# re-ovo/wgpu-path-tracing

Measured on AMD Instinct MI355X. Metric: Msamples/s (rays x bounces / s), higher is better.
Workload: dtype f32

## Files before the change

### include/ptmi.h

```cpp
#ifndef PTMI_H
#define PTMI_H

#include <stddef.h>
#include <stdint.h>
#include "ptmi_layout.h"

#ifdef __cplusplus
extern "C" {
#endif

#define PTMI_ABI_VERSION 4

enum {
    PTMI_OK = 0,
    PTMI_E_INVALID = -1,
    PTMI_E_NODEVICE = -2,
    PTMI_E_HIP = -3,
    PTMI_E_STATE = -4,
    PTMI_E_UNSUPPORTED = -5
};

enum { PTMI_ATLAS_RGBA16F = 1, PTMI_ATLAS_RGBA32F = 2 };
enum { PTMI_TRAVERSAL_AUTO = 0, PTMI_TRAVERSAL_GLOBAL = 1, PTMI_TRAVERSAL_LDS = 2, PTMI_TRAVERSAL_GLOBAL_EXACT = 3 };

// ... 370 lines not shown
int ptmi_multi_alpha_status(ptmi_multi *m, struct ptmi_alpha_status *out);

typedef struct ptmi_alpha_blend_params {
    uint32_t max_layers;
    uint32_t seed;
    uint32_t reserved[2];
} ptmi_alpha_blend_params;
struct ptmi_alpha_blend_status {
    uint32_t present, n_materials, n_blend, max_layers, seed, reserved;
    uint64_t path_tests, path_passes, shadow_tests, shadow_passes;
};
int ptmi_set_alpha_blend(ptmi_ctx *ctx, const float *factor, uint32_t n_materials, const ptmi_alpha_blend_params *params );
int ptmi_alpha_blend_status(ptmi_ctx *ctx, struct ptmi_alpha_blend_status *out);
int ptmi_multi_set_alpha_blend(ptmi_multi *m, const float *factor, uint32_t n_materials, const ptmi_alpha_blend_params *params);
int ptmi_multi_alpha_blend_status(ptmi_multi *m, struct ptmi_alpha_blend_status *out);

int ptmi_get_stats(ptmi_ctx *ctx, ptmi_stats *out);
int ptmi_reset_stats(ptmi_ctx *ctx);

int ptmi_debug_raygen(ptmi_ctx *ctx, const ptmi_camera *camera, uint32_t n, const uint32_t *xs,
                      const uint32_t *ys, const uint32_t *frames, float *o3, float *d3, uint32_t *rng);
int ptmi_debug_center_rays(ptmi_ctx *ctx, const ptmi_camera *camera, float *o3, float *d3, size_t n_floats_each);
int ptmi_debug_intersect(ptmi_ctx *ctx, uint32_t n, const float *o3, const float *d3,
                         float *t, uint32_t *tri, float *u, float *v);
int ptmi_debug_occluded(ptmi_ctx *ctx, uint32_t n, const float *o3, const float *d3,
                        const float *dist, uint8_t *occluded);
int ptmi_debug_alpha_intersect(ptmi_ctx *ctx, uint32_t n, const float *o3, const float *d3, float *t, uint32_t *tri, uint32_t *layers);
int ptmi_debug_alpha_occluded(ptmi_ctx *ctx, uint32_t n, const float *o3, const float *d3, const float *dist, uint8_t *occluded,
                              uint32_t *layers);
int ptmi_debug_image_stats(const ptmi_triangle *triangles, uint32_t n_triangles,
// ... 33 lines not shown
```

### wgpu-path-tracing_amd/csrc/dispatch.hip

```cpp
#include "ptmi_ctx.h"

#include <algorithm>
#include <cmath>
#include <cstring>
#include <utility>
#include <vector>

namespace {

constexpr size_t kMaxPendingEvents = 4096;
constexpr size_t kMaxDispatchesInFlight = 256;

const struct { double ptmi_stats::*ms; uint64_t ptmi_stats::*launches; } kEventStat[kEventKinds] = {
    {&ptmi_stats::gpu_ms, nullptr},
    {&ptmi_stats::extend_ms, &ptmi_stats::extend_launches},
    {&ptmi_stats::shade_ms, &ptmi_stats::shade_launches},
    {&ptmi_stats::shadow_ms, &ptmi_stats::shadow_launches},
    {&ptmi_stats::raygen_ms, nullptr},
    {&ptmi_stats::compact_ms, nullptr},
    {&ptmi_stats::accumulate_ms, nullptr},
};

hipEvent_t get_event(ptmi_ctx *c) {
    if (!c->event_pool.empty()) { hipEvent_t e = c->event_pool.back(); c->event_pool.pop_back(); return e; }
// ... 50 lines not shown
}

struct Timed {
    ptmi_ctx *c; hipEvent_t a = nullptr, b = nullptr; EventKind kind; bool on;
    hipStream_t st;
    Timed(ptmi_ctx *c_, EventKind kind_, bool on_, hipStream_t st_ = nullptr) : c(c_), kind(kind_), on(on_), st(st_ ? st_ : c_->stream) {
        if (on) { a = get_event(c); b = get_event(c); (void)hipEventRecord(a, st); }
    }
    ~Timed() {
        if (!on) return;
        (void)hipEventRecord(b, st);
        c->pending.push_back({a, b, kind});
        if (c->pending.size() > kMaxPendingEvents) drain_completed_events(c);
    }
};

#ifndef PT_REPACK
#define PT_REPACK 1
#endif

int dispatch(ptmi_ctx *c, const ptmi_camera *cam, uint32_t n_frames, const ptmi_adaptive_params *ap, uint32_t rounds,
             const DevFlagMap *map = nullptr, bool count_call = true, const ListedRays *listed = nullptr) {
    int rc = check_ready(c, true);
    if (rc) return rc;
    uint32_t proj = PTMI_PROJ_PERSPECTIVE;
    if (!listed) {
        if (!cam) return fail(c, PTMI_E_INVALID, "camera is NULL");
        if (cam->width != c->W || cam->height != c->H)
            return fail(c, PTMI_E_INVALID, "camera says %ux%u but the output buffer is %ux%u", cam->width, cam->height, c->W, c->H);
        if ((rc = pt_check_camera(c, cam, &proj, c->err))) return rc;
// ... 27 lines not shown
    if (npix * F > 0xFFFFFF00ull) return fail(c, PTMI_E_UNSUPPORTED, "batch of %llu paths exceeds 2^32", (unsigned long long)(npix * F));
    TraverseConfig cfg, cfg_shadow;
    if ((rc = traverse_pick(c, true, cfg)) || (rc = traverse_pick(c, false, cfg_shadow))) return rc;
    for (;;) {
        rc = ensure_capacity(c, ln, (size_t)(npix * F), depth);
        if (rc == PTMI_OK) break;
        if (!auto_F || !c->alloc_oom || F <= 1) return rc;
        F = (F + 1) / 2;
    }
    if ((rc = traverse_arm(c, true, kSpillMain, cfg, true)) || (rc = traverse_arm(c, false, side ? kSpillSide : kSpillAfterExtend, cfg_shadow, true)))
        return rc;
    c->st.traversal_used = pt_variant(cfg.variant).where == PT_FROM_MEMORY ? PTMI_TRAVERSAL_GLOBAL : PTMI_TRAVERSAL_LDS;
    c->st.frames_per_batch_used = F;
    c->st.radiance_stride_bytes = (walks_memory_quantised(cfg) || walks_memory_quantised(cfg_shadow)) ? 16u : 12u;
    c->st.shade_tables = PT_SHADE_LDS_BUDGET | ((uint32_t)pt_shade_stage(c->sc.n_mats, c->sc.n_lights) << 28);
    const int blocks = c->n_cu * 8;
#ifndef PT_SHADE_WGS_PER_CU
#define PT_SHADE_WGS_PER_CU 16
#endif
    const int shade_blocks = c->n_cu * PT_SHADE_WGS_PER_CU;
    const uint32_t maxb = c->opt.max_bounces;
    const bool t1 = c->opt.timing >= 1, t2 = c->opt.timing >= 2, t3 = c->opt.timing >= 3;
    {
        Timed td(c, kDispatch, t1);
        const hipStream_t ms = c->stream;
        const hipStream_t ss = side ? ln.side : ms;
        const int tiles = (int)(ln.cap / pt_compact_tile_slots() + 1);
        ln.paths.l_stride = c->st.radiance_stride_bytes / 4u;
        DevPaths bp = ln.paths;
        if (!env_w) bp.W = nullptr;
        const uint32_t rb = PT_REPACK ? pt_repack_bounce() : 0xFFFFFFFEu;
        DevPaths tp = ln.tail;
        tp.L = bp.L; tp.l_stride = bp.l_stride;
        if (!env_w) tp.W = nullptr;
        float4 *const aov_rec = c->aov_mask || depth ? ln.aov : nullptr;
        float4 *const mom = plane_as<float4>(c, kMoments);
        unsigned long long *const ct = c->d_counters;
        uint32_t *const qlen = &c->d_control[kCwQueue], *const slen = &c->d_control[kCwShadow];
        if (ap && !map && first_frame == 0u) { pt_launch_adaptive_restart(ms, blocks, band, mom); c->ad_rounds = 0; }
        const DevRays rays = listed ? listed->rays : DevRays{CameraSource{cam, proj}};
        auto batch = [&](uint32_t frame0, uint32_t fb) -> int {
            const DevPixels px = ap     ? DevPixels{ListedPixels{band, c->ad.list, &c->d_control[kCwAdActive], mom, &ct[kCtAdTraced]}}
                                 : listed ? DevPixels{BakedPixels{band, listed->list, listed->count, frame0}}
                                          : DevPixels{DensePixels{band, frame0}};
            { Timed t(c, kRaygen, t3, ms); pt_launch_raygen(ms, blocks, rays, px, fb, bp, &qlen[0]); }
            int cur = 0;
            for (uint32_t b = 0; b < maxb; b++) {
                const bool tail = b > rb;
                const uint32_t *q = b == 0 || b == rb + 1 ? nullptr : ln.queue[cur];
                const DevPaths sp = tail ? tp : bp;
                const int par = side ? (int)(b & 1u) : 0;
                const ShadeParams shp{b, maxb, c->opt.do_mis, ln.counts, side ? 1u : 0u, tail ? ln.pid : nullptr};
                { Timed t(c, kExtend, t2, ms); launch_extend(c, ms, cfg, sp, q, &qlen[b], ln.hits);
                  if (alpha) alpha_resolve_paths(c, ms, cfg, sp, q, &qlen[b], ln.hits, nullptr); }
                const bool last = b + 1 == maxb;
                if (side && b >= 2) HIP_TRY(c, hipStreamWaitEvent(ms, ln.ev_shadow[par], 0));
                { Timed t(c, kShade, t3, ms);
                  (c->opt.perf_mode ? pt_launch_shade_fast : pt_launch_shade)(
// ... 37 lines not shown
            }
            c->ad_rounds += rounds;
        } else {
            for (uint32_t f0 = 0; f0 < n_frames; f0 += F)
                if ((rc = batch(first_frame + f0, std::min(F, n_frames - f0)))) return rc;
        }
    }
    HIP_TRY(c, hipGetLastError());
    {
        hipEvent_t done = get_event(c);
        HIP_TRY(c, hipEventRecord(done, c->stream));
        c->in_flight.push_back(done);
        if (c->in_flight.size() > kMaxDispatchesInFlight) HIP_TRY(c, throttle(c, kMaxDispatchesInFlight));
    }
    if (!ap) { c->st.paths += npix * n_frames; c->st.frames += n_frames; }
    if (count_call) c->st.dispatches += 1;
    return PTMI_OK;
}

}

int pt_adaptive_check(ptmi_ctx *c, const ptmi_camera *cam, const ptmi_adaptive_params *params, ptmi_adaptive_params *out) {
    if (!c) return PTMI_E_INVALID;
    if (!params) return fail(c, PTMI_E_INVALID, "params is NULL");
    ptmi_adaptive_params ap = *params;
    if (!(ap.threshold > 0.0f)) return fail(c, PTMI_E_INVALID, "threshold %g is not > 0", (double)ap.threshold);
    if (!(ap.floor >= 0.0f) || std::isinf(ap.floor)) return fail(c, PTMI_E_INVALID, "floor %g is negative or not finite", (double)ap.floor);
    if (ap.reserved[0] || ap.reserved[1]) return fail(c, PTMI_E_INVALID, "a reserved word of ptmi_adaptive_params is not zero");
    if (ap.neighbourhood > 1u) return fail(c, PTMI_E_INVALID, "neighbourhood %u is not 0 or 1", ap.neighbourhood);
    if (ap.floor == 0.0f) ap.floor = 1.0f;
// ... 47 lines not shown
}

int ptmi_dispatch_bake(ptmi_ctx *c, const ptmi_bake_params *params, uint32_t n_frames) {
    ptmi_bake_params bp;
    const int rc = bake_check(c, params, &bp);
    if (rc) return rc;
    const ListedRays listed{BakeSurface{c->d_bake_texels, bp.bias}, c->d_bake_covered, c->bake_covered, bp.first_frame};
    return dispatch(c, nullptr, n_frames, nullptr, 0, nullptr, true, &listed);
}

int ptmi_dispatch_probes(ptmi_ctx *c, const ptmi_probe_params *params, uint32_t n_frames) {
    ListedRays listed;
    const int rc = probes_check(c, params, &listed);
    if (rc) return rc;
    return dispatch(c, nullptr, n_frames, nullptr, 0, nullptr, true, &listed);
}

int ptmi_adaptive_status(ptmi_ctx *c, struct ptmi_adaptive_status *out) {
    if (!c || !out) return PTMI_E_INVALID;
    if (!c->moments_on) return fail(c, PTMI_E_STATE, "the moments plane is off (ptmi_set_moments)");
    if (!c->plane[kMoments]) return fail(c, PTMI_E_STATE, "no output buffer (ptmi_resize)");
    HIP_TRY(c, hipSetDevice(c->device));
    std::memset(out, 0, sizeof *out);
    const DevBand band = pt_band_of(c->opt, c->W, c->H);
    const unsigned long long preset[3] = {0ull, ~0ull, 0ull};
    unsigned long long sum_min_max[3] = {0ull, 0ull, 0ull};
    uint32_t active = 0u;
    HIP_TRY(c, quiesce(c));
    if (band.y0 < band.y1 && band.rows) {
        HIP_TRY(c, hipMemcpyAsync(&c->d_counters[kCtAdSum], preset, sizeof preset, hipMemcpyHostToDevice, c->stream));
// ... 118 lines not shown
```

### wgpu-path-tracing_amd/csrc/pipeline.hip

```cpp
#include "pt_ballot_list.h"
#include "pt_device.h"
#include "pt_math.h"

#include <cstdlib>
#include <type_traits>

namespace {

constexpr int BLOCK = 256;

template <int PROJ>
PT_DEV v3 camera_dir(const ptmi_camera &cam, float px, float py, v3 &org0) {
    float uvx = (px / (float)cam.width) * 2.0f - 1.0f;
    float uvy = (py / (float)cam.height) * 2.0f - 1.0f;
    v3 fw = mk3(cam.forward[0], cam.forward[1], cam.forward[2]);
    v3 rt = mk3(cam.right[0], cam.right[1], cam.right[2]);
    v3 up = mk3(cam.up[0], cam.up[1], cam.up[2]);
    org0 = mk3(cam.position[0], cam.position[1], cam.position[2]);
    if constexpr (PROJ == (int)PTMI_PROJ_ORTHOGRAPHIC) {
        const float ymag = __uint_as_float(cam._p3[1]);
        v3 a = scale3(scale3(scale3(rt, uvx), ymag), cam.aspect);
        v3 b = scale3(scale3(up, uvy), ymag);
        org0 = add3(add3(org0, a), b);
        return normalize3(fw);
// ... 89 lines not shown
    const float4 *__restrict__ probes; uint32_t shift, cols, count;
    PT_DEV void ray(uint32_t x, uint32_t y, uint32_t frame, size_t, v3 &o, v3 &d, uint32_t &rng) const {
        const uint32_t i = (y >> shift) * cols + (x >> shift);
        o = d = mk3(0.0f, 0.0f, 0.0f); rng = 0u;
        if ((x >> shift) >= cols || i >= count) return;
        const float4 p = probes[i];
        if (__float_as_uint(p.w) != 0u) probe_ray(p, 1u << shift, x, y, frame, o, d, rng);
    }
};

template <class Rays, class Pixels>
PT_DEV void raygen(const Rays &rays, const Pixels &px, uint32_t n_frames, DevPaths P, uint32_t *__restrict__ count_out) {
    const DevBand &band = px.band;
    const uint32_t n = px.entries();
    const uint32_t total = n * n_frames;
    if (blockIdx.x == 0 && threadIdx.x == 0) { px.count_paths(total); *count_out = total; }
    for (uint32_t p = blockIdx.x * BLOCK + threadIdx.x; p < total; p += gridDim.x * BLOCK) {
        const uint32_t k = p / n, pix = px.pixel(p - k * n);
        const uint32_t y = band.row_of(pix / band.width), x = pix % band.width;
        const size_t fp = (size_t)y * band.width + x;
        v3 o, d; uint32_t rng;
        rays.ray(x, y, px.first_frame(fp) + k, fp, o, d, rng);
        init_path(P, p, o, d, rng);
    }
}
template <class Rays, class Pixels>
__global__ __launch_bounds__(BLOCK) void k_first_rays(Rays rays, Pixels px, uint32_t n_frames, DevPaths P, uint32_t *__restrict__ count_out) {
    raygen(rays, px, n_frames, P, count_out);
}
template <class Rays>
__global__ __launch_bounds__(BLOCK) void k_first_rays_list(Rays rays, uint32_t width, uint32_t n, const uint32_t *xs, const uint32_t *ys,
// ... 95 lines not shown
        const float t = 1.0f / (float)(frame + 1u);
        for (int i = 0; i < N; i++) acc[i] = mix1(acc[i], x[i], t);
    } else {
        for (int i = 0; i < N; i++) acc[i] = x[i];
    }
}
PT_DEV rgb_sc ld_clamped(const float *__restrict__ L, uint32_t l_stride, size_t p) {
    rgb_sc l;
    if (l_stride == 4u) { const float4 v = reinterpret_cast<const float4 *>(L)[p]; l = rgb_sc{v.x, v.y, v.z}; }
    else l = reinterpret_cast<const rgb_sc *>(L)[p];
    return rgb_sc{min1(l.x, 2.5f), min1(l.y, 2.5f), min1(l.z, 2.5f)};
}

template <class Pixels>
PT_DEV void fold_radiance(const Pixels &px, uint32_t n_frames, const float *__restrict__ L, uint32_t l_stride, float4 *__restrict__ out) {
    const uint32_t n = px.entries();
    for (uint32_t j = blockIdx.x * BLOCK + threadIdx.x; j < n; j += gridDim.x * BLOCK) {
        const size_t oi = px.band.frame_pixel(px.pixel(j));
        const uint32_t frame0 = px.first_frame(oi);
        const float4 o = out[oi];
        float acc[3] = {o.x, o.y, o.z};
        for (uint32_t k = 0; k < n_frames; k++) {
            const rgb_sc c = ld_clamped(L, l_stride, (size_t)k * n + j);
            fold(acc, {c.x, c.y, c.z}, frame0 + k);
        }
        out[oi] = n_frames ? make_float4(acc[0], acc[1], acc[2], 0.0f) : o;
    }
}

template <class Pixels>
PT_DEV void fold_aov(const Pixels &px, uint32_t n_frames, const float4 *__restrict__ rec, const ptmi_triangle *__restrict__ tris,
                     uint32_t n_tris, float4 *__restrict__ albedo, float4 *__restrict__ normal, uint2 *__restrict__ ids) {
    const uint32_t n = px.entries();
    for (uint32_t j = blockIdx.x * BLOCK + threadIdx.x; j < n; j += gridDim.x * BLOCK) {
        const size_t oi = px.band.frame_pixel(px.pixel(j));
        const uint32_t frame0 = px.first_frame(oi);
        const float4 a = albedo ? albedo[oi] : make_float4(0.0f, 0.0f, 0.0f, 0.0f);
        const float4 nm = normal ? normal[oi] : make_float4(0.0f, 0.0f, 0.0f, 0.0f);
// ... 356 lines not shown
        hipLaunchKernelGGL(k_scatter_packed, dim3(tiles), dim3(TILE_WORDS), 0, s, count, shadow_mask, shadow_sums, shadow_queue,
                           shadow_count, st);
}
void pt_launch_repack(hipStream_t s, int blocks, const uint32_t *count, const uint32_t *queue, DevPaths from, DevPaths to,
                      uint32_t *pid) {
    hipLaunchKernelGGL(k_repack, dim3(blocks), dim3(BLOCK), 0, s, count, queue, from, to, pid);
}
void pt_launch_accumulate(hipStream_t s, int blocks, const DevPixels &px, uint32_t n_frames, const float *L, uint32_t l_stride, float4 *out) {
    std::visit([&](auto src) {
        hipLaunchKernelGGL(k_fold_radiance<decltype(src)>, dim3(blocks), dim3(BLOCK), 0, s, src, n_frames, L, l_stride, out);
    }, px);
}
void pt_launch_accumulate_aov(hipStream_t s, int blocks, const DevPixels &px, uint32_t n_frames, const float4 *rec,
                              const ptmi_triangle *tris, uint32_t n_tris, float4 *albedo, float4 *normal, uint2 *ids) {
    std::visit([&](auto src) {
        if constexpr (std::is_same_v<decltype(src), BakedPixels>) abort();
        else hipLaunchKernelGGL(k_fold_aov<decltype(src)>, dim3(blocks), dim3(BLOCK), 0, s, src, n_frames, rec, tris, n_tris, albedo, normal, ids);
    }, px);
}
void pt_launch_accumulate_probe_depth(hipStream_t s, int blocks, const DevPixels &px, uint32_t n_frames, const float4 *rec, float max_distance,
                                      float4 *plane) {
    std::visit([&](auto src) {
        if constexpr (std::is_same_v<decltype(src), BakedPixels>)
            hipLaunchKernelGGL(k_fold_probe_depth<BakedPixels>, dim3(blocks), dim3(BLOCK), 0, s, src, n_frames, rec, max_distance, plane);
        else abort();
    }, px);
}
void pt_launch_accumulate_moments(hipStream_t s, int blocks, const DevPixels &px, uint32_t n_frames, const float *L, uint32_t l_stride,
                                  float4 *mom) {
    std::visit([&](auto src) {
        hipLaunchKernelGGL(k_fold_moments<decltype(src)>, dim3(blocks), dim3(BLOCK), 0, s, src, n_frames, L, l_stride, mom);
    }, px);
}
void pt_launch_adaptive_restart(hipStream_t s, int blocks, DevBand band, float4 *mom) {
    hipLaunchKernelGGL(k_ad_restart, dim3(blocks), dim3(BLOCK), 0, s, band, mom);
}
void pt_launch_adaptive_list(hipStream_t s, int blocks, DevBand band, const ptmi_adaptive_params &ap, const float4 *mom,
                             const DevFlagMap *fm, DevAdaptive ad) {
    const int tiles = (int)pt_adaptive_tiles(band.rows * band.width);
    uint32_t *const n_pixels = &ad.control[kCwAdPixels];
    if (fm) hipLaunchKernelGGL(k_ad_select_map, dim3(blocks), dim3(BLOCK), 0, s, band, ap, mom, *fm, ad.ballot, ad.control);
    else hipLaunchKernelGGL(k_ad_select, dim3(blocks), dim3(BLOCK), 0, s, band, ap, mom, ad.ballot, ad.control);
    hipLaunchKernelGGL(k_ad_tile_sums, dim3(tiles), dim3(TILE_WORDS), 0, s, n_pixels, ad.ballot, ad.tile_sums);
    hipLaunchKernelGGL(k_ad_scatter, dim3(tiles), dim3(TILE_WORDS), 0, s, n_pixels, ad.ballot, ad.tile_sums, ad.list, &ad.control[kCwAdActive]);
}
void pt_launch_adaptive_flags(hipStream_t s, int blocks, DevBand band, const ptmi_adaptive_params &ap, const float4 *mom, uint8_t *flags) {
// ... 22 lines not shown
```

### wgpu-path-tracing_amd/csrc/pt_device.h

```cpp
#pragma once
#include <hip/hip_runtime.h>
#include <stdint.h>
#include <initializer_list>
#include <variant>
#include "ptmi_layout.h"
#include "ptmi.h"

#define PT_HD __host__ __device__ inline

#define PT_REF_LEAF      0x80000000u
#define PT_REF_NONE      0xFFFFFFFFu
#define PT_LEAF_MAX_TRIS 32u
#define PT_LEAF_OFF_BITS 26u
#define PT_LEAF_OFF_MASK ((1u << PT_LEAF_OFF_BITS) - 1u)

struct DevEnv {
    const float4 *tab;
    const uint2 *alias;
    uint32_t w, h;
    uint32_t sampled;
    float intensity, rotation;
};

struct DevMedium {
// ... 203 lines not shown
    int wants_spill;
    int quantized;
};
inline uint32_t pt_variant_code(const TraverseConfig &cfg) { return (uint32_t)cfg.variant * 10u + (uint32_t)cfg.wgs_per_cu; }
#ifndef PT_QCACHE_NODES
#define PT_QCACHE_NODES 256
#endif
#define PT_SPILL_ENTRIES 64
size_t pt_spill_bytes(int blocks);

struct DensePixels {
    DevBand band; uint32_t frame0;
    __device__ uint32_t entries() const { return band.rows * band.width; }
    __device__ uint32_t pixel(uint32_t j) const { return j; }
    __device__ uint32_t first_frame(size_t) const { return frame0; }
    __device__ void count_paths(uint32_t) const {}
};
struct ListedPixels {
    DevBand band; const uint32_t *list, *n_active; const float4 *mom;
    unsigned long long *traced;
    __device__ uint32_t entries() const { return *n_active; }
    __device__ uint32_t pixel(uint32_t j) const { return list[j]; }
    __device__ uint32_t first_frame(size_t oi) const { return (uint32_t)mom[oi].z; }
    __device__ void count_paths(uint32_t paths) const { atomicAdd(traced, (unsigned long long)paths); }
};
struct BakedPixels {
    DevBand band; const uint32_t *covered; uint32_t n, frame0;
    __device__ uint32_t entries() const { return n; }
    __device__ uint32_t pixel(uint32_t j) const { return covered[j]; }
    __device__ uint32_t first_frame(size_t) const { return frame0; }
    __device__ void count_paths(uint32_t) const {}
};
using DevPixels = std::variant<DensePixels, ListedPixels, BakedPixels>;
struct CameraSource { const ptmi_camera *cam; uint32_t proj; };
struct BakeSurface { const float4 *texels; float bias; };
struct ProbeSet { const float4 *probes; uint32_t shift, cols, count; };
using DevRays = std::variant<CameraSource, BakeSurface, ProbeSet>;
void pt_launch_raygen(hipStream_t s, int blocks, const DevRays &rays, const DevPixels &px, uint32_t n_frames, DevPaths p, uint32_t *count_out);
void pt_launch_raygen_list(hipStream_t s, const DevRays &rays, uint32_t width, uint32_t n, const uint32_t *xs, const uint32_t *ys,
                           const uint32_t *frames, DevPaths p);
float4 *pt_launch_bake_dilate(hipStream_t s, uint32_t W, uint32_t H, uint32_t passes, const float4 *texels, const float4 *out,
                              float4 *a, float4 *b);
struct DevProbeAtlas { const float4 *out; const float4 *probes; uint32_t W, shift, cols, count; };
void pt_launch_probe_sh(hipStream_t s, DevProbeAtlas a, const float *basis9, float *sh);
size_t pt_probe_irradiance_lds(uint32_t shift);
void pt_launch_probe_irradiance(hipStream_t s, DevProbeAtlas a, const float4 *dir_dw, const float4 *normals, uint32_t m, float4 *irr);
void pt_launch_probe_visibility(hipStream_t s, DevProbeAtlas depth, const float4 *dir_dw, const float4 *normals, uint32_t m, uint32_t sharpness_log2,
                                uint32_t border, float4 *vis);
// ... 107 lines not shown
```

### wgpu-path-tracing_amd/csrc/ptmi_api.hip

```cpp
#include "ptmi_ctx.h"

#include <algorithm>
#include <cmath>
#include <cstdarg>
#include <cstdio>
#include <cstring>

namespace {

void vfail(std::string &err, const char *fmt, va_list ap) {
    char buf[512];
    vsnprintf(buf, sizeof buf, fmt, ap);
    err = buf;
}

constexpr size_t kLaneBytes[kLaneBufs] = {
    16, 16, 8, 16,
    8,
    16 + 16 + sizeof(rgb_sc), 4, 16 + 16 + sizeof(rgb_sc), 4,
    16, 16, 8, 4,
    4, 4,
    1,
    32,
    4, 4,
// ... 248 lines not shown
#else
        ok = ok && hipStreamCreateWithPriority(&ln.side, hipStreamNonBlocking, hi) == hipSuccess;
#endif
        for (hipEvent_t *e : {&ln.ev_ready, &ln.ev_shadow[0], &ln.ev_shadow[1]})
            ok = ok && hipEventCreateWithFlags(e, hipEventDisableTiming) == hipSuccess;
        if (!ok) { ptmi_destroy(c); return fail(nullptr, PTMI_E_HIP, "stream / event creation failed"); }
    }
    if (hipMalloc(&c->d_counters, kCounterWords * sizeof(unsigned long long)) != hipSuccess ||
        hipMalloc(&c->d_control, kControlWords * sizeof(uint32_t)) != hipSuccess ||
        hipMalloc(&c->d_scene, sizeof(DevScene)) != hipSuccess || hipMemset(c->d_scene, 0, sizeof(DevScene)) != hipSuccess ||
        hipMemset(c->d_counters, 0, kCounterWords * sizeof(unsigned long long)) != hipSuccess ||
        hipMemset(c->d_control, 0, kControlWords * sizeof(uint32_t)) != hipSuccess) {
        ptmi_destroy(c); return fail(nullptr, PTMI_E_HIP, "device allocation failed");
    }
    c->ad.control = c->d_control; c->ad.counters = c->d_counters;
    *out = c;
    return PTMI_OK;
}

int ptmi_destroy(ptmi_ctx *c) {
    if (!c) return PTMI_E_INVALID;
    (void)hipSetDevice(c->device);
    (void)sync_all(c);
    drain_events(c);
    for (hipEvent_t e : c->in_flight) (void)hipEventDestroy(e);
    for (hipEvent_t e : c->event_pool) (void)hipEventDestroy(e);
    {
        Lane &ln = c->lane;
        free_batch(ln);
        dfree(ln.d_spill); dfree(ln.d_spill_side);
// ... 342 lines not shown
    for (int i = 0; i < kMaxBounces; i++) c->st.segments_by_bounce[i] = h[kCtByBounce + i];
    c->st.verify_failed = h[kCtVerifyFailed];
    c->st.bvh_depth = stats_depth(c);
    *out = c->st;
    out->paths += h[kCtAdTraced];
    return PTMI_OK;
}

int ptmi_reset_stats(ptmi_ctx *c) {
    if (!c) return PTMI_E_INVALID;
    HIP_TRY(c, hipSetDevice(c->device));
    HIP_TRY(c, quiesce(c));
    HIP_TRY(c, hipMemset(c->d_counters, 0, kCtDispatchEnd * sizeof(unsigned long long)));
    const ptmi_stats old = c->st;
    std::memset(&c->st, 0, sizeof c->st);
    c->st.bvh_depth = stats_depth(c);
    c->st.upload_ms = old.upload_ms; c->st.upload_tree_ms = old.upload_tree_ms; c->st.upload_copy_ms = old.upload_copy_ms;
    c->st.leaves_used = old.leaves_used; c->st.leaf_tris_used = old.leaf_tris_used; c->st.tree_builder_used = old.tree_builder_used;
    return PTMI_OK;
}

}
```

### wgpu-path-tracing_amd/csrc/ptmi_ctx.h

```cpp
#pragma once
#include "ptmi.h"
#include "pt_device.h"

#include <chrono>
#include <cmath>
#include <cstddef>
#include <cstdint>
#include <deque>
#include <string>
#include <vector>

struct ptmi_ctx;
struct PtPrepared;
PtPrepared *pt_prepare_scene(ptmi_ctx *c, const ptmi_triangle *tris, uint32_t nt, const ptmi_material *mats, uint32_t nm,
                             const ptmi_bvh_node *nodes, uint32_t nn, const ptmi_light *lights, uint32_t nl, int *rc_out);
int pt_install_scene(ptmi_ctx *c, PtPrepared *p);
void pt_free_prepared(PtPrepared *p);
int pt_atlas_bytes(uint32_t width, uint32_t height, int format, size_t *bytes, char *why, size_t why_len);
int pt_check_medium(const ptmi_medium *m, std::string &err);
int pt_check_medium_depth(const ptmi_medium *m, std::string &err);
int pt_check_medium_density(const float *rho, uint32_t nx, uint32_t ny, uint32_t nz, const ptmi_medium_grid *params,
                            struct ptmi_medium_grid_status *st, std::string &err);
const ptmi_medium *pt_ctx_medium(const ptmi_ctx *c);
bool pt_ctx_has_medium_grid(const ptmi_ctx *c);
// ... 174 lines not shown
    uint32_t *d_bake_covered = nullptr;
    uint32_t bake_covered = 0;
    float4 *d_probes = nullptr;
    uint32_t *d_probe_list = nullptr;
    float4 *d_probe_dir_dw = nullptr;
    float *d_probe_basis = nullptr;
    float4 *d_probe_normals = nullptr;
    struct ptmi_probe_status probe{};
    bool probe_depth_on = false;
    ptmi_probe_depth_params probe_depth{};
    unsigned long long *d_counters = nullptr;
    uint32_t *d_control = nullptr;
    DevAdaptive ad{};
    uint32_t ad_rounds = 0;

    ptmi_stats st{};
    std::vector<EventPair> pending;
    std::vector<hipEvent_t> event_pool;
    std::deque<hipEvent_t> in_flight;
};

PT_HOST {

extern thread_local std::string g_create_err;
int fail(std::string &err, int code, const char *fmt, ...);
int fail(const ptmi_ctx *c, int code, const char *fmt, ...);
#define HIP_TRY(c, expr) do { hipError_t e_ = (expr); if (e_ != hipSuccess) \
    return fail((c), PTMI_E_HIP, "%s failed: %s (%s:%d)", #expr, hipGetErrorString(e_), __FILE__, __LINE__); } while (0)

template <class T> void dfree(T *&p) { if (p) { (void)hipFree(p); p = nullptr; } }
// ... 105 lines not shown
```

### wgpu-path-tracing_amd/ptmi/native.py

```python
import ctypes
import functools
import os
import types

import numpy as np

from . import layout

_LIB_DIR = os.path.join(os.path.dirname(os.path.dirname(os.path.abspath(__file__))), "lib")
LIB_PATH = os.environ.get("PTMI_LIB") or os.path.join(_LIB_DIR, "libptmi.so")

TRAVERSAL_AUTO, TRAVERSAL_GLOBAL, TRAVERSAL_LDS, TRAVERSAL_GLOBAL_EXACT = 0, 1, 2, 3
ATLAS_RGBA16F, ATLAS_RGBA32F = 1, 2

EXPORTS = [
    "ptmi_abi_version", "ptmi_create", "ptmi_destroy", "ptmi_last_error", "ptmi_upload_scene",
    "ptmi_upload_atlas", "ptmi_resize", "ptmi_set_options", "ptmi_get_options", "ptmi_dispatch",
    "ptmi_synchronize", "ptmi_read_output", "ptmi_write_output", "ptmi_output_device_ptr",
    "ptmi_bind_output_device", "ptmi_set_stream", "ptmi_blit", "ptmi_get_stats", "ptmi_reset_stats",
    "ptmi_debug_raygen", "ptmi_debug_intersect", "ptmi_debug_occluded", "ptmi_debug_math", "ptmi_debug_exact_math", "ptmi_get_size",
    "ptmi_debug_image_stats", "ptmi_debug_build_image", "ptmi_debug_read_image", "ptmi_throttle", "ptmi_multi_throttle",
    "ptmi_multi_create", "ptmi_multi_destroy", "ptmi_multi_last_error", "ptmi_multi_count", "ptmi_multi_context",
    "ptmi_multi_upload_scene", "ptmi_multi_upload_atlas", "ptmi_multi_resize", "ptmi_multi_set_options", "ptmi_multi_get_options",
    "ptmi_multi_dispatch", "ptmi_multi_gather", "ptmi_multi_synchronize", "ptmi_multi_read_output", "ptmi_multi_write_output",
# ... 17 lines not shown
    "ptmi_multi_update_triangles", "ptmi_multi_update_materials", "ptmi_multi_update_lights", "ptmi_multi_scene_update_status",
    "ptmi_rebuild_tree", "ptmi_rebuild_status", "ptmi_multi_rebuild_tree", "ptmi_multi_rebuild_status",
    "ptmi_set_alpha_cutoff", "ptmi_alpha_status", "ptmi_multi_set_alpha_cutoff", "ptmi_multi_alpha_status",
    "ptmi_debug_alpha_intersect", "ptmi_debug_alpha_occluded",
    "ptmi_set_alpha_blend", "ptmi_alpha_blend_status", "ptmi_multi_set_alpha_blend", "ptmi_multi_alpha_blend_status",
    "ptmi_set_triangle_groups", "ptmi_transform_groups", "ptmi_transform_status", "ptmi_normal_matrix", "ptmi_debug_read_triangles",
    "ptmi_multi_set_triangle_groups", "ptmi_multi_transform_groups", "ptmi_multi_transform_status",
    "ptmi_set_skin", "ptmi_pose_skin", "ptmi_skin_status", "ptmi_multi_set_skin", "ptmi_multi_pose_skin", "ptmi_multi_skin_status",
    "ptmi_set_morph", "ptmi_pose_morph", "ptmi_morph_status", "ptmi_multi_set_morph", "ptmi_multi_pose_morph", "ptmi_multi_morph_status",
    "ptmi_set_projections", "ptmi_get_projections", "ptmi_multi_set_projections", "ptmi_multi_get_projections",
    "ptmi_upload_bake_surface", "ptmi_dispatch_bake", "ptmi_bake_status", "ptmi_bake_dilate", "ptmi_debug_bake_rays",
    "ptmi_upload_probes", "ptmi_dispatch_probes", "ptmi_probe_status", "ptmi_probe_sh", "ptmi_probe_irradiance",
    "ptmi_debug_probe_rays", "ptmi_debug_probe_tables",
    "ptmi_set_probe_depth", "ptmi_get_probe_depth", "ptmi_read_probe_depth", "ptmi_write_probe_depth", "ptmi_probe_depth_device_ptr",
    "ptmi_probe_visibility",
]
MULTI_LOOPBACK = 1
MULTI_PLANE_MOMENTS, MULTI_PLANE_OUTPUT = 0x100, 0x200
AOV_ALBEDO, AOV_NORMAL, AOV_ID = 1, 2, 4
AOVS = {"albedo": (AOV_ALBEDO, np.float32, 4), "normal": (AOV_NORMAL, np.float32, 4), "id": (AOV_ID, np.uint32, 2)}
ABI_VERSION = 4


class PtmiError(RuntimeError):
    def __init__(self, code, msg):
        super().__init__(f"ptmi error {code}: {msg}")
        self.code = code


class Options(ctypes.Structure):
    _fields_ = [("max_bounces", ctypes.c_uint32), ("do_mis", ctypes.c_uint32),
# ... 197 lines not shown

class ProbeStatus(ctypes.Structure):
    _fields_ = [("present", ctypes.c_uint32), ("tile", ctypes.c_uint32), ("count", ctypes.c_uint32), ("enabled", ctypes.c_uint32),
                ("texels", ctypes.c_uint32)]

    def as_dict(self):
        return {n: int(getattr(self, n)) for n, _ in self._fields_}


class ProbeDepthParams(ctypes.Structure):
    _fields_ = [("max_distance", ctypes.c_float), ("reserved", ctypes.c_uint32 * 3)]


class ProbeVisibilityParams(ctypes.Structure):
    _fields_ = [("m", ctypes.c_uint32), ("sharpness_log2", ctypes.c_uint32), ("border", ctypes.c_uint32), ("reserved", ctypes.c_uint32)]


class Stats(ctypes.Structure):
    _fields_ = [("paths", ctypes.c_uint64), ("segments", ctypes.c_uint64), ("shadow_rays", ctypes.c_uint64),
                ("dispatches", ctypes.c_uint64), ("frames", ctypes.c_uint64),
                ("segments_by_bounce", ctypes.c_uint64 * 64),
                ("gpu_ms", ctypes.c_double), ("extend_ms", ctypes.c_double), ("extend_launches", ctypes.c_uint64),
                ("shade_ms", ctypes.c_double), ("shadow_ms", ctypes.c_double),
                ("bvh_depth", ctypes.c_uint32), ("traversal_used", ctypes.c_uint32),
                ("frames_per_batch_used", ctypes.c_uint32), ("radiance_stride_bytes", ctypes.c_uint32),
                ("shadow_traced", ctypes.c_uint64), ("shade_launches", ctypes.c_uint64), ("shadow_launches", ctypes.c_uint64),
                ("raygen_ms", ctypes.c_double), ("compact_ms", ctypes.c_double), ("accumulate_ms", ctypes.c_double),
                ("upload_ms", ctypes.c_double), ("upload_tree_ms", ctypes.c_double), ("upload_copy_ms", ctypes.c_double),
                ("leaves_used", ctypes.c_uint32), ("leaf_tris_used", ctypes.c_uint32),
                ("extend_variant", ctypes.c_uint32), ("shadow_variant", ctypes.c_uint32), ("verify_failed", ctypes.c_uint64),
# ... 124 lines not shown
        L.ptmi_debug_medium_density.argtypes = [vp, u32, vp, vp]
        L.ptmi_debug_medium_grid_check.argtypes = [vp, vp, u32, u32, u32, vp, vp]
        L.ptmi_debug_medium_track.argtypes = [vp, u32, vp, vp, vp, vp, u32, vp, vp, vp, vp, vp]
        L.ptmi_debug_alpha_intersect.argtypes = [vp, u32, vp, vp, vp, vp, vp]
        L.ptmi_debug_alpha_occluded.argtypes = [vp, u32, vp, vp, vp, vp, vp]
        L.ptmi_normal_matrix.restype = None
        L.ptmi_normal_matrix.argtypes = [vp, vp]
        L.ptmi_debug_read_triangles.argtypes = [vp, u32, u32, vp]
        for name, args in list(_BAKE.items()) + list(_PROBES.items()):
            if name in EXPORTS:
                getattr(L, name).argtypes = [vp] + args
        if "ptmi_debug_probe_tables" in EXPORTS:
            L.ptmi_debug_probe_tables.argtypes = [u32, vp, vp]
        if "ptmi_probe_depth_device_ptr" in EXPORTS:
            L.ptmi_probe_depth_device_ptr.restype = vp
        _lib = L
    return _lib


def _p(a):
    return a.ctypes.data_as(ctypes.c_void_p) if a is not None else None


def image_stats(scene):
    L = load()
    out = (ctypes.c_double * 8)()
    rc = L.ptmi_debug_image_stats(_p(scene.tris), len(scene.tris), _p(scene.nodes), len(scene.nodes), out)
    if rc != 0:
        raise PtmiError(rc, L.ptmi_last_error(None).decode())
    keys = ("wide_nodes", "leaves", "depth", "quantised_nodes", "stream_dwords", "containment_violations",
# ... 467 lines not shown
    def moments_device_ptr(self):
        return self.L.ptmi_moments_device_ptr(self.h)

    def denoised_device_ptr(self):
        return self.L.ptmi_denoised_device_ptr(self.h)

    def dispatch_adaptive(self, camera, rounds=1, threshold=0.0, floor=0.0, min_frames=0, max_frames=0, step=0, neighbourhood=0,
                          reserved=(0, 0)):
        self._dispatch_adaptive(camera, rounds, threshold, floor, min_frames, max_frames, step, neighbourhood, reserved)

    def reproject(self, from_cam, to_cam, max_history=0, depth_tolerance=0.0, match_ids=0, reserved=(0, 0, 0, 0, 0)):
        assert from_cam.dtype == layout.CAMERA and to_cam.dtype == layout.CAMERA
        prm = ReprojectParams(max_history, depth_tolerance, match_ids, (ctypes.c_uint32 * 5)(*reserved))
        self._ck(self.L.ptmi_reproject(self.h, _p(from_cam), _p(to_cam), ctypes.byref(prm)))

    def reproject_status(self):
        st = ReprojectStatus()
        self._ck(self.L.ptmi_reproject_status(self.h, ctypes.byref(st)))
        return st

    def debug_center_rays(self, camera):
        n = self.width * self.height
        o, d = np.zeros((n, 3), np.float32), np.zeros((n, 3), np.float32)
        self._ck(self.L.ptmi_debug_center_rays(self.h, _p(camera), _p(o), _p(d), o.size))
        return o, d

    @staticmethod
    def _bake_params(first_frame, bias, reserved):
        if first_frame == 0 and bias is None and tuple(reserved) == (0, 0):
            return None
# ... 305 lines not shown
```

Measured before the change: 12830.

## Skip primary rays outside the projected scene bounds with a frame scissor

On the host, the scene's root bounding box is projected through the perspective camera, conservatively padded for box error, lens aperture and pixel margins. When there is no environment map, medium, AOV, moments or alpha, only pixels inside that screen rectangle are generated, traced and shaded. The fold kernel writes zero radiance for pixels outside it, and the skipped paths are still added to the segment counters as single missed segments. This removes traversal and shading for rays that must miss the scene, at the cost of host-side projection work, a wider fold pass, and a correctness risk if the bound is ever not conservative.

```diff
diff --git a/include/ptmi.h b/include/ptmi.h
--- a/include/ptmi.h
+++ b/include/ptmi.h
@@ -408,6 +408,27 @@
 int ptmi_alpha_blend_status(ptmi_ctx *ctx, struct ptmi_alpha_blend_status *out);
 int ptmi_multi_set_alpha_blend(ptmi_multi *m, const float *factor, uint32_t n_materials, const ptmi_alpha_blend_params *params);
 int ptmi_multi_alpha_blend_status(ptmi_multi *m, struct ptmi_alpha_blend_status *out);
+
+enum {
+    PTMI_SCISSOR_APPLIED = 0,
+    PTMI_SCISSOR_OFF = 1,
+    PTMI_SCISSOR_NOT_PLAIN = 2,
+    PTMI_SCISSOR_ENVIRONMENT = 3,
+    PTMI_SCISSOR_MEDIUM = 4,
+    PTMI_SCISSOR_AOV = 5,
+    PTMI_SCISSOR_MOMENTS = 6,
+    PTMI_SCISSOR_ALPHA = 7,
+    PTMI_SCISSOR_PROJECTION = 8,
+    PTMI_SCISSOR_NO_PROMISE = 9,
+    PTMI_SCISSOR_NOTHING = 10
+};
+struct ptmi_scissor_status {
+    uint32_t x0, x1, y0, y1;
+    uint32_t applied;
+    uint32_t reason;
+    uint64_t skipped;
+};
+int ptmi_scissor_status(ptmi_ctx *ctx, struct ptmi_scissor_status *out);
 
 int ptmi_get_stats(ptmi_ctx *ctx, ptmi_stats *out);
 int ptmi_reset_stats(ptmi_ctx *ctx);
diff --git a/wgpu-path-tracing_amd/csrc/dispatch.hip b/wgpu-path-tracing_amd/csrc/dispatch.hip
--- a/wgpu-path-tracing_amd/csrc/dispatch.hip
+++ b/wgpu-path-tracing_amd/csrc/dispatch.hip
@@ -1,4 +1,5 @@
 #include "ptmi_ctx.h"
+#include "scene/frame_scissor.h"
 
 #include <algorithm>
 #include <cmath>
@@ -88,6 +89,39 @@
         if (c->pending.size() > kMaxPendingEvents) drain_completed_events(c);
     }
 };
+
+struct ScissorRect { uint32_t l0, l1, x0, x1; };
+bool frame_scissor(ptmi_ctx *c, const ptmi_camera *cam, uint32_t proj, const DevBand &band, bool plain, ScissorRect &r) {
+    struct ptmi_scissor_status &st = c->scissor;
+    st.x0 = 0u; st.x1 = c->W; st.y0 = 0u; st.y1 = c->H; st.applied = 0u;
+    const auto no = [&](uint32_t reason) { st.reason = reason; return false; };
+    if (!c->scissor_on) return no(PTMI_SCISSOR_OFF);
+    if (!plain) return no(PTMI_SCISSOR_NOT_PLAIN);
+    if (c->sc.env.tab) return no(PTMI_SCISSOR_ENVIRONMENT);
+    if (c->sc.med.on) return no(PTMI_SCISSOR_MEDIUM);
+    if (c->aov_mask) return no(PTMI_SCISSOR_AOV);
+    if (c->plane[kMoments]) return no(PTMI_SCISSOR_MOMENTS);
+    if (alpha_active(c)) return no(PTMI_SCISSOR_ALPHA);
+    if (proj != PTMI_PROJ_PERSPECTIVE) return no(PTMI_SCISSOR_PROJECTION);
+    if (c->sc.root_ref == PT_REF_NONE) return no(PTMI_SCISSOR_NO_PROMISE);
+    float lo[3], hi[3];
+    for (int k = 0; k < 3; k++) {
+        lo[k] = std::min(c->sc.root_min[k], c->sc.ref_root_min[k]);
+        hi[k] = std::max(c->sc.root_max[k], c->sc.ref_root_max[k]);
+    }
+    ptmi_camera pin = *cam;
+    ptmi_camera_set_projection(&pin, PTMI_PROJ_PERSPECTIVE, 0.0f);
+    const int why = pt_frame_scissor(&pin, lo, hi, &st.x0, &st.x1, &st.y0, &st.y1);
+    if (why != PT_SCISSOR_RECT) return no(why == PT_SCISSOR_PROJECTION ? PTMI_SCISSOR_PROJECTION : PTMI_SCISSOR_NO_PROMISE);
+    r.l0 = 0u;
+    while (r.l0 < band.rows && band.row_of(r.l0) < st.y0) r.l0++;
+    r.l1 = r.l0;
+    while (r.l1 < band.rows && band.row_of(r.l1) < st.y1) r.l1++;
+    r.x0 = st.x0; r.x1 = st.x1;
+    if (r.l0 == 0u && r.l1 == band.rows && r.x0 == 0u && r.x1 == band.width) return no(PTMI_SCISSOR_NOTHING);
+    st.reason = PTMI_SCISSOR_APPLIED; st.applied = 1u;
+    return true;
+}
 
 #ifndef PT_REPACK
 #define PT_REPACK 1
@@ -145,6 +179,9 @@
     c->st.frames_per_batch_used = F;
     c->st.radiance_stride_bytes = (walks_memory_quantised(cfg) || walks_memory_quantised(cfg_shadow)) ? 16u : 12u;
     c->st.shade_tables = PT_SHADE_LDS_BUDGET | ((uint32_t)pt_shade_stage(c->sc.n_mats, c->sc.n_lights) << 28);
+    ScissorRect sr{};
+    const bool scissored = frame_scissor(c, cam, proj, band, !ap && !listed, sr);
+    const uint64_t skipped_px = scissored ? npix - (uint64_t)(sr.l1 - sr.l0) * (sr.x1 - sr.x0) : 0u;
     const int blocks = c->n_cu * 8;
 #ifndef PT_SHADE_WGS_PER_CU
 #define PT_SHADE_WGS_PER_CU 16
@@ -173,6 +210,7 @@
         auto batch = [&](uint32_t frame0, uint32_t fb) -> int {
             const DevPixels px = ap     ? DevPixels{ListedPixels{band, c->ad.list, &c->d_control[kCwAdActive], mom, &ct[kCtAdTraced]}}
                                  : listed ? DevPixels{BakedPixels{band, listed->list, listed->count, frame0}}
+                                 : scissored ? DevPixels{ScissoredPixels{band, sr.l0, sr.l1, sr.x0, sr.x1, frame0, ct}}
                                           : DevPixels{DensePixels{band, frame0}};
             { Timed t(c, kRaygen, t3, ms); pt_launch_raygen(ms, blocks, rays, px, fb, bp, &qlen[0]); }
             int cur = 0;
@@ -240,6 +278,7 @@
         if (c->in_flight.size() > kMaxDispatchesInFlight) HIP_TRY(c, throttle(c, kMaxDispatchesInFlight));
     }
     if (!ap) { c->st.paths += npix * n_frames; c->st.frames += n_frames; }
+    c->scissor.skipped += skipped_px * n_frames;
     if (count_call) c->st.dispatches += 1;
     return PTMI_OK;
 }
@@ -317,6 +356,12 @@
     const int rc = probes_check(c, params, &listed);
     if (rc) return rc;
     return dispatch(c, nullptr, n_frames, nullptr, 0, nullptr, true, &listed);
+}
+
+int ptmi_scissor_status(ptmi_ctx *c, struct ptmi_scissor_status *out) {
+    if (!c || !out) return PTMI_E_INVALID;
+    *out = c->scissor;
+    return PTMI_OK;
 }
 
 int ptmi_adaptive_status(ptmi_ctx *c, struct ptmi_adaptive_status *out) {
diff --git a/wgpu-path-tracing_amd/csrc/pipeline.hip b/wgpu-path-tracing_amd/csrc/pipeline.hip
--- a/wgpu-path-tracing_amd/csrc/pipeline.hip
+++ b/wgpu-path-tracing_amd/csrc/pipeline.hip
@@ -127,7 +127,7 @@
     const DevBand &band = px.band;
     const uint32_t n = px.entries();
     const uint32_t total = n * n_frames;
-    if (blockIdx.x == 0 && threadIdx.x == 0) { px.count_paths(total); *count_out = total; }
+    if (blockIdx.x == 0 && threadIdx.x == 0) { px.count_paths(total, n_frames); *count_out = total; }
     for (uint32_t p = blockIdx.x * BLOCK + threadIdx.x; p < total; p += gridDim.x * BLOCK) {
         const uint32_t k = p / n, pix = px.pixel(p - k * n);
         const uint32_t y = band.row_of(pix / band.width), x = pix % band.width;
@@ -253,14 +253,20 @@
 
 template <class Pixels>
 PT_DEV void fold_radiance(const Pixels &px, uint32_t n_frames, const float *__restrict__ L, uint32_t l_stride, float4 *__restrict__ out) {
+    constexpr bool SCISSORED = std::is_same_v<Pixels, ScissoredPixels>;
     const uint32_t n = px.entries();
-    for (uint32_t j = blockIdx.x * BLOCK + threadIdx.x; j < n; j += gridDim.x * BLOCK) {
-        const size_t oi = px.band.frame_pixel(px.pixel(j));
+    uint32_t walk = n;
+    if constexpr (SCISSORED) walk = px.band.rows * px.band.width;
+    for (uint32_t j = blockIdx.x * BLOCK + threadIdx.x; j < walk; j += gridDim.x * BLOCK) {
+        uint32_t pix = j, e = j;
+        if constexpr (SCISSORED) e = px.fold_entry(j); else pix = px.pixel(j);
+        const size_t oi = px.band.frame_pixel(pix);
         const uint32_t frame0 = px.first_frame(oi);
         const float4 o = out[oi];
         float acc[3] = {o.x, o.y, o.z};
         for (uint32_t k = 0; k < n_frames; k++) {
-            const rgb_sc c = ld_clamped(L, l_stride, (size_t)k * n + j);
+            rgb_sc c{0.0f, 0.0f, 0.0f};
+            if (!SCISSORED || e != ScissoredPixels::kOutside) c = ld_clamped(L, l_stride, (size_t)k * n + e);
             fold(acc, {c.x, c.y, c.z}, frame0 + k);
         }
         out[oi] = n_frames ? make_float4(acc[0], acc[1], acc[2], 0.0f) : o;
@@ -647,7 +653,7 @@
 void pt_launch_accumulate_aov(hipStream_t s, int blocks, const DevPixels &px, uint32_t n_frames, const float4 *rec,
                               const ptmi_triangle *tris, uint32_t n_tris, float4 *albedo, float4 *normal, uint2 *ids) {
     std::visit([&](auto src) {
-        if constexpr (std::is_same_v<decltype(src), BakedPixels>) abort();
+        if constexpr (std::is_same_v<decltype(src), BakedPixels> || std::is_same_v<decltype(src), ScissoredPixels>) abort();
         else hipLaunchKernelGGL(k_fold_aov<decltype(src)>, dim3(blocks), dim3(BLOCK), 0, s, src, n_frames, rec, tris, n_tris, albedo, normal, ids);
     }, px);
 }
@@ -662,7 +668,8 @@
 void pt_launch_accumulate_moments(hipStream_t s, int blocks, const DevPixels &px, uint32_t n_frames, const float *L, uint32_t l_stride,
                                   float4 *mom) {
     std::visit([&](auto src) {
-        hipLaunchKernelGGL(k_fold_moments<decltype(src)>, dim3(blocks), dim3(BLOCK), 0, s, src, n_frames, L, l_stride, mom);
+        if constexpr (std::is_same_v<decltype(src), ScissoredPixels>) abort();
+        else hipLaunchKernelGGL(k_fold_moments<decltype(src)>, dim3(blocks), dim3(BLOCK), 0, s, src, n_frames, L, l_stride, mom);
     }, px);
 }
 void pt_launch_adaptive_restart(hipStream_t s, int blocks, DevBand band, float4 *mom) {
diff --git a/wgpu-path-tracing_amd/csrc/pt_device.h b/wgpu-path-tracing_amd/csrc/pt_device.h
--- a/wgpu-path-tracing_amd/csrc/pt_device.h
+++ b/wgpu-path-tracing_amd/csrc/pt_device.h
@@ -241,7 +241,23 @@
     __device__ uint32_t entries() const { return band.rows * band.width; }
     __device__ uint32_t pixel(uint32_t j) const { return j; }
     __device__ uint32_t first_frame(size_t) const { return frame0; }
-    __device__ void count_paths(uint32_t) const {}
+    __device__ void count_paths(uint32_t, uint32_t) const {}
+};
+struct ScissoredPixels {
+    DevBand band; uint32_t l0, l1, x0, x1, frame0;
+    unsigned long long *stats;
+    __device__ uint32_t entries() const { return (l1 - l0) * (x1 - x0); }
+    __device__ uint32_t pixel(uint32_t j) const { const uint32_t w = x1 - x0; return (l0 + j / w) * band.width + x0 + j % w; }
+    __device__ uint32_t first_frame(size_t) const { return frame0; }
+    __device__ void count_paths(uint32_t, uint32_t n_frames) const {
+        const unsigned long long skipped = (unsigned long long)(band.rows * band.width - entries()) * n_frames;
+        atomicAdd(&stats[kCtSegments], skipped); atomicAdd(&stats[kCtByBounce], skipped);
+    }
+    static constexpr uint32_t kOutside = 0xFFFFFFFFu;
+    __device__ uint32_t fold_entry(uint32_t pix) const {
+        const uint32_t l = pix / band.width, x = pix % band.width;
+        return l >= l0 && l < l1 && x >= x0 && x < x1 ? (l - l0) * (x1 - x0) + (x - x0) : kOutside;
+    }
 };
 struct ListedPixels {
     DevBand band; const uint32_t *list, *n_active; const float4 *mom;
@@ -249,16 +265,16 @@
     __device__ uint32_t entries() const { return *n_active; }
     __device__ uint32_t pixel(uint32_t j) const { return list[j]; }
     __device__ uint32_t first_frame(size_t oi) const { return (uint32_t)mom[oi].z; }
-    __device__ void count_paths(uint32_t paths) const { atomicAdd(traced, (unsigned long long)paths); }
+    __device__ void count_paths(uint32_t paths, uint32_t) const { atomicAdd(traced, (unsigned long long)paths); }
 };
 struct BakedPixels {
     DevBand band; const uint32_t *covered; uint32_t n, frame0;
     __device__ uint32_t entries() const { return n; }
     __device__ uint32_t pixel(uint32_t j) const { return covered[j]; }
     __device__ uint32_t first_frame(size_t) const { return frame0; }
-    __device__ void count_paths(uint32_t) const {}
-};
-using DevPixels = std::variant<DensePixels, ListedPixels, BakedPixels>;
+    __device__ void count_paths(uint32_t, uint32_t) const {}
+};
+using DevPixels = std::variant<DensePixels, ListedPixels, BakedPixels, ScissoredPixels>;
 struct CameraSource { const ptmi_camera *cam; uint32_t proj; };
 struct BakeSurface { const float4 *texels; float bias; };
 struct ProbeSet { const float4 *probes; uint32_t shift, cols, count; };
diff --git a/wgpu-path-tracing_amd/csrc/ptmi_api.hip b/wgpu-path-tracing_amd/csrc/ptmi_api.hip
--- a/wgpu-path-tracing_amd/csrc/ptmi_api.hip
+++ b/wgpu-path-tracing_amd/csrc/ptmi_api.hip
@@ -4,6 +4,7 @@
 #include <cmath>
 #include <cstdarg>
 #include <cstdio>
+#include <cstdlib>
 #include <cstring>
 
 namespace {
@@ -286,6 +287,7 @@
         ptmi_destroy(c); return fail(nullptr, PTMI_E_HIP, "device allocation failed");
     }
     c->ad.control = c->d_control; c->ad.counters = c->d_counters;
+    if (const char *e = std::getenv("PTMI_SCISSOR")) c->scissor_on = std::strcmp(e, "0") != 0;
     *out = c;
     return PTMI_OK;
 }
@@ -658,6 +660,7 @@
     HIP_TRY(c, hipMemset(c->d_counters, 0, kCtDispatchEnd * sizeof(unsigned long long)));
     const ptmi_stats old = c->st;
     std::memset(&c->st, 0, sizeof c->st);
+    c->scissor.skipped = 0;
     c->st.bvh_depth = stats_depth(c);
     c->st.upload_ms = old.upload_ms; c->st.upload_tree_ms = old.upload_tree_ms; c->st.upload_copy_ms = old.upload_copy_ms;
     c->st.leaves_used = old.leaves_used; c->st.leaf_tris_used = old.leaf_tris_used; c->st.tree_builder_used = old.tree_builder_used;
diff --git a/wgpu-path-tracing_amd/csrc/ptmi_ctx.h b/wgpu-path-tracing_amd/csrc/ptmi_ctx.h
--- a/wgpu-path-tracing_amd/csrc/ptmi_ctx.h
+++ b/wgpu-path-tracing_amd/csrc/ptmi_ctx.h
@@ -212,6 +212,9 @@
     DevAdaptive ad{};
     uint32_t ad_rounds = 0;
 
+    bool scissor_on = true;
+    struct ptmi_scissor_status scissor{};
+
     ptmi_stats st{};
     std::vector<EventPair> pending;
     std::vector<hipEvent_t> event_pool;
diff --git a/wgpu-path-tracing_amd/csrc/scene/frame_scissor.cpp b/wgpu-path-tracing_amd/csrc/scene/frame_scissor.cpp
--- /dev/null
+++ b/wgpu-path-tracing_amd/csrc/scene/frame_scissor.cpp
@@ -0,0 +1,109 @@
+#include "frame_scissor.h"
+
+#include <algorithm>
+#include <cmath>
+
+namespace {
+
+struct d3 { double x, y, z; };
+d3 sub(d3 a, d3 b) { return {a.x - b.x, a.y - b.y, a.z - b.z}; }
+d3 cross(d3 a, d3 b) { return {a.y * b.z - a.z * b.y, a.z * b.x - a.x * b.z, a.x * b.y - a.y * b.x}; }
+double dot(d3 a, d3 b) { return a.x * b.x + a.y * b.y + a.z * b.z; }
+d3 of(const float v[3]) { return {(double)v[0], (double)v[1], (double)v[2]}; }
+bool finite3(const float v[3]) { return std::isfinite(v[0]) && std::isfinite(v[1]) && std::isfinite(v[2]); }
+
+struct p2 { double x, y; };
+
+constexpr double kPixelMargin = 2.0;
+constexpr double kClipMargin = 1.0 / 16.0;
+constexpr uint32_t kMaxSide = 65536u;
+constexpr double kBoxMargin = 1.0 / 65536.0;
+constexpr double kFront = 1e-6;
+constexpr double kMaxFov = 3.0;
+
+void pixel_range(double pmin, double pmax, uint32_t n, uint32_t &lo, uint32_t &hi) {
+    const double a = std::floor(std::max(pmin, -8.0)) - kPixelMargin, b = std::floor(std::min(pmax, (double)n + 8.0)) + 1.0 + kPixelMargin;
+    lo = (uint32_t)std::min(std::max(a, 0.0), (double)n);
+    hi = (uint32_t)std::min(std::max(b, 0.0), (double)n);
+}
+
+}
+
+extern "C" int pt_frame_scissor(const ptmi_camera *cam, const float box_min[3], const float box_max[3],
+                                uint32_t *x0, uint32_t *x1, uint32_t *y0, uint32_t *y1) {
+    const uint32_t W = cam->width, H = cam->height;
+    *x0 = 0u; *x1 = W; *y0 = 0u; *y1 = H;
+    if (W == 0u || H == 0u) return PT_SCISSOR_NOT_FINITE;
+    if (W > kMaxSide || H > kMaxSide) return PT_SCISSOR_DEGENERATE;
+    if (!finite3(cam->position) || !finite3(cam->forward) || !finite3(cam->right) || !finite3(cam->up) || !std::isfinite(cam->fov) ||
+        !std::isfinite(cam->aspect) || !std::isfinite(cam->aperture) || !std::isfinite(cam->focus_distance) || !finite3(box_min) ||
+        !finite3(box_max))
+        return PT_SCISSOR_NOT_FINITE;
+    if (ptmi_camera_projection(cam) != PTMI_PROJ_PERSPECTIVE) return PT_SCISSOR_PROJECTION;
+    d3 lo = of(box_min), hi = of(box_max);
+    if (lo.x > hi.x || lo.y > hi.y || lo.z > hi.z) return PT_SCISSOR_NOT_FINITE;
+    if (!(cam->fov > 0.0f) || (double)cam->fov > kMaxFov || !(cam->aspect > 0.0f)) return PT_SCISSOR_DEGENERATE;
+    const double th = std::tan((double)cam->fov * 0.5), tx = th * (double)cam->aspect;
+    const d3 pos = of(cam->position), fw = of(cam->forward), rt = of(cam->right), up = of(cam->up);
+
+    double big = 0.0;
+    for (double v : {lo.x, lo.y, lo.z, hi.x, hi.y, hi.z}) big = std::max(big, std::fabs(v));
+    double grow = big * kBoxMargin;
+    auto corner = [&](int i, double g) { return d3{(i & 1 ? hi.x + g : lo.x - g), (i & 2 ? hi.y + g : lo.y - g), (i & 4 ? hi.z + g : lo.z - g)}; };
+    if (cam->aperture > 0.0f) {
+        const double r2 = dot(rt, rt), u2 = dot(up, up);
+        const double A = (double)cam->aperture * std::sqrt(std::max(r2, u2) + std::fabs(dot(rt, up)));
+        const double f = (double)cam->focus_distance;
+        if (!(f > A)) return PT_SCISSOR_DEGENERATE;
+        double D = 0.0;
+        for (int i = 0; i < 8; i++) { const d3 q = sub(corner(i, grow), pos); D = std::max(D, std::sqrt(dot(q, q))); }
+        grow += A * std::max(1.0, (D - f) / (f - A));
+    }
+    if (!std::isfinite(grow)) return PT_SCISSOR_NOT_FINITE;
+    lo = corner(0, grow); hi = corner(7, grow);
+    if (pos.x >= lo.x && pos.x <= hi.x && pos.y >= lo.y && pos.y <= hi.y && pos.z >= lo.z && pos.z <= hi.z) return PT_SCISSOR_INSIDE;
+
+    const d3 c_s = cross(rt, up), c_u = cross(up, fw), c_v = cross(fw, rt);
+    const double det = dot(fw, c_s);
+    const double scale = std::sqrt(dot(fw, fw) * dot(rt, rt) * dot(up, up));
+    if (!(scale > 0.0) || !(std::fabs(det) > 1e-6 * scale)) return PT_SCISSOR_DEGENERATE;
+    const double fwl = std::sqrt(dot(fw, fw));
+    p2 at[8];
+    for (int i = 0; i < 8; i++) {
+        const d3 q = sub(corner(i, grow), pos);
+        const double s = dot(q, c_s) / det, u = dot(q, c_u) / det, v = dot(q, c_v) / det;
+        if (!(s * fwl > kFront * std::sqrt(dot(q, q)))) return PT_SCISSOR_BEHIND;
+        at[i] = {(u / s / tx + 1.0) * 0.5 * (double)W, (v / s / th + 1.0) * 0.5 * (double)H};
+        if (!std::isfinite(at[i].x) || !std::isfinite(at[i].y)) return PT_SCISSOR_NOT_FINITE;
+    }
+    static const int kFaces[6][4] = {{0, 2, 6, 4}, {1, 3, 7, 5}, {0, 1, 5, 4}, {2, 3, 7, 6}, {0, 1, 3, 2}, {4, 5, 7, 6}};
+    double pxmin = INFINITY, pxmax = -INFINITY, pymin = INFINITY, pymax = -INFINITY;
+    for (const auto &face : kFaces) {
+        p2 poly[16], next[16];
+        int n = 4;
+        for (int k = 0; k < 4; k++) poly[k] = at[face[k]];
+        for (int e = 0; e < 4 && n > 0; e++) {
+            const bool is_x = e < 2;
+            const double sign = (e & 1) ? 1.0 : -1.0, bound = (e & 1) ? (double)(is_x ? W : H) + kClipMargin : kClipMargin;
+            auto dist = [&](p2 p) { return sign * (is_x ? p.x : p.y) - bound; };
+            int m = 0;
+            for (int k = 0; k < n; k++) {
+                const p2 a = poly[k], b = poly[(k + 1) % n];
+                const double da = dist(a), db = dist(b);
+                if (da <= 0.0) next[m++] = a;
+                if ((da <= 0.0) != (db <= 0.0)) { const double t = da / (da - db); next[m++] = {a.x + t * (b.x - a.x), a.y + t * (b.y - a.y)}; }
+            }
+            n = m;
+            for (int k = 0; k < n; k++) poly[k] = next[k];
+        }
+        for (int k = 0; k < n; k++) {
+            pxmin = std::min(pxmin, poly[k].x); pxmax = std::max(pxmax, poly[k].x);
+            pymin = std::min(pymin, poly[k].y); pymax = std::max(pymax, poly[k].y);
+        }
+    }
+    if (!(pxmin <= pxmax)) { *x0 = *x1 = *y0 = *y1 = 0u; return PT_SCISSOR_RECT; }
+    pixel_range(pxmin, pxmax, W, *x0, *x1);
+    pixel_range(pymin, pymax, H, *y0, *y1);
+    if (*x0 >= *x1 || *y0 >= *y1) *x0 = *x1 = *y0 = *y1 = 0u;
+    return PT_SCISSOR_RECT;
+}
diff --git a/wgpu-path-tracing_amd/csrc/scene/frame_scissor.h b/wgpu-path-tracing_amd/csrc/scene/frame_scissor.h
--- /dev/null
+++ b/wgpu-path-tracing_amd/csrc/scene/frame_scissor.h
@@ -0,0 +1,21 @@
+#pragma once
+#include <stdint.h>
+#include "ptmi_layout.h"
+
+enum {
+    PT_SCISSOR_RECT = 0,
+    PT_SCISSOR_NOT_FINITE = 1,
+    PT_SCISSOR_PROJECTION = 2,
+    PT_SCISSOR_INSIDE = 3,
+    PT_SCISSOR_BEHIND = 4,
+    PT_SCISSOR_DEGENERATE = 5,
+};
+
+#ifdef __cplusplus
+extern "C" {
+#endif
+int pt_frame_scissor(const ptmi_camera *cam, const float box_min[3], const float box_max[3],
+                     uint32_t *x0, uint32_t *x1, uint32_t *y0, uint32_t *y1);
+#ifdef __cplusplus
+}
+#endif
diff --git a/wgpu-path-tracing_amd/ptmi/native.py b/wgpu-path-tracing_amd/ptmi/native.py
--- a/wgpu-path-tracing_amd/ptmi/native.py
+++ b/wgpu-path-tracing_amd/ptmi/native.py
@@ -55,7 +55,10 @@
     "ptmi_debug_probe_rays", "ptmi_debug_probe_tables",
     "ptmi_set_probe_depth", "ptmi_get_probe_depth", "ptmi_read_probe_depth", "ptmi_write_probe_depth", "ptmi_probe_depth_device_ptr",
     "ptmi_probe_visibility",
+    "ptmi_scissor_status",
 ]
+(SCISSOR_APPLIED, SCISSOR_OFF, SCISSOR_NOT_PLAIN, SCISSOR_ENVIRONMENT, SCISSOR_MEDIUM, SCISSOR_AOV, SCISSOR_MOMENTS, SCISSOR_ALPHA,
+ SCISSOR_PROJECTION, SCISSOR_NO_PROMISE, SCISSOR_NOTHING) = range(11)
 MULTI_LOOPBACK = 1
 MULTI_PLANE_MOMENTS, MULTI_PLANE_OUTPUT = 0x100, 0x200
 AOV_ALBEDO, AOV_NORMAL, AOV_ID = 1, 2, 4
@@ -283,6 +286,14 @@
 
 class ProbeVisibilityParams(ctypes.Structure):
     _fields_ = [("m", ctypes.c_uint32), ("sharpness_log2", ctypes.c_uint32), ("border", ctypes.c_uint32), ("reserved", ctypes.c_uint32)]
+
+
+class ScissorStatus(ctypes.Structure):
+    _fields_ = [("x0", ctypes.c_uint32), ("x1", ctypes.c_uint32), ("y0", ctypes.c_uint32), ("y1", ctypes.c_uint32),
+                ("applied", ctypes.c_uint32), ("reason", ctypes.c_uint32), ("skipped", ctypes.c_uint64)]
+
+    def as_dict(self):
+        return {n: int(getattr(self, n)) for n, _ in self._fields_}
 
 
 class Stats(ctypes.Structure):
@@ -437,6 +448,8 @@
             L.ptmi_debug_probe_tables.argtypes = [u32, vp, vp]
         if "ptmi_probe_depth_device_ptr" in EXPORTS:
             L.ptmi_probe_depth_device_ptr.restype = vp
+        if "ptmi_scissor_status" in EXPORTS:
+            L.ptmi_scissor_status.argtypes = [vp, vp]
         _lib = L
     return _lib
 
@@ -934,6 +947,11 @@
         prm = ReprojectParams(max_history, depth_tolerance, match_ids, (ctypes.c_uint32 * 5)(*reserved))
         self._ck(self.L.ptmi_reproject(self.h, _p(from_cam), _p(to_cam), ctypes.byref(prm)))
 
+    def scissor_status(self):
+        st = ScissorStatus()
+        self._ck(self.L.ptmi_scissor_status(self.h, ctypes.byref(st)))
+        return st
+
     def reproject_status(self):
         st = ReprojectStatus()
         self._ck(self.L.ptmi_reproject_status(self.h, ctypes.byref(st)))
```

Measured after the change: 13480, median of 6. 1.05x the previous value.
